# grisetti/g2o_frontend

Hardware: AMD Instinct MI355X
Metric: depth-pair alignments/sec (640x480, 10 GN iters) (higher is better)
Workload: dtype f32; 1 GPU; loop-closure batch: 128 independent 640x480 depth pairs per GPU (u16 mm frames resident in HBM; per pair: convert 2 frames + Aligner::align, 10x1 GN iterations); BASELINE configs[3] shard; mode=pairs, pairs_per_gpu=128, total_pairs=128, rows=480, cols=640, sub_frames=64, sub_pairs=64, streams=4, omega_storage=sym6, step_mode=fused, parallelism=independent pairs sharded over 1 GPU(s), RCCL all-gather of result records only

## Files before the change

### g2o_frontend_amd/csrc/pwn_hip_capi.hip

```cpp
#include <cstdlib>
#include "../../include/pwn_hip.h"
#include "../../include/pwn_hip_testing.h"
#include "pwn_buffers.h"
#include "pwn_kernels.h"
#include "pwn_scene_kernels.h"
#include "pwn_stats.h"

#include <algorithm>
#include <chrono>
#include <condition_variable>
#include <functional>
#include <cstddef>
#include <cstdio>
#include <cstring>
#include <map>
#include <mutex>
#include <string>
#include <thread>
#include <type_traits>
#include <vector>

using namespace pwnhip;

namespace {
// ... 438 lines not shown
  HIPCHK(ctx, ctx->state_host.ensure(B), PWN_HIP_ERR_ALLOCATION);
  HIPCHK(ctx, ctx->counts_host.ensure(B + 1), PWN_HIP_ERR_ALLOCATION);
  HIPCHK(ctx, ctx->match_dev.ensure(B), PWN_HIP_ERR_ALLOCATION);
  HIPCHK(ctx, ctx->match_host.ensure(B), PWN_HIP_ERR_ALLOCATION);
  HIPCHK(ctx, ctx->stats_dev.ensure(B), PWN_HIP_ERR_ALLOCATION);
  HIPCHK(ctx, ctx->stats_host.ensure(B), PWN_HIP_ERR_ALLOCATION);
  ctx->desc_cap = (int)B;
  return PWN_HIP_OK;
}

constexpr int kSinglePassMinFrames = 16;
void launch_stats(const ConvertParams& cp, const FrameDesc* fr, int n, hipStream_t st) {
  const unsigned perFrame = (unsigned)cp.rows * (unsigned)((cp.cols + 255) / 256);
  const unsigned nblk = (n >= 8 ? 8u * (unsigned)((n + 7) / 8) : (unsigned)n) * perFrame;
  hipLaunchKernelGGL(k_stats, dim3(nblk), dim3(256), 0, st, fr, cp, n);
}
int launch_front_end(pwn_hip_ctx* ctx, const ConvertParams& cp, int base, int n, hipStream_t st, bool single_pass, int* fault_out) {
  const FrameDesc* fr = ctx->frames_dev + base;
  if (single_pass) {
    { StageTimer t(ctx, "unproject", st);
      const bool raw = ctx->frames_host[base].raw != nullptr;
      bool aligned = cp.cols % (raw ? 8 : 4) == 0;
      for (int i = 0; i < n && aligned; ++i) {
        const FrameDesc& fd = ctx->frames_host[base + i];
        aligned = ((uintptr_t)(raw ? (const void*)fd.raw : (const void*)fd.depth) & 15u) == 0;
      }
      if (aligned && raw) hipLaunchKernelGGL(k_strip_count<true>, dim3((cp.rows + 3) / 4, n), dim3(256), 0, st, fr, cp);
      else if (aligned) hipLaunchKernelGGL(k_strip_count<false>, dim3((cp.rows + 3) / 4, n), dim3(256), 0, st, fr, cp);
      else hipLaunchKernelGGL(k_strip_count_any, dim3(cp.rows, n), dim3(256), 0, st, fr, cp);
      hipLaunchKernelGGL(k_row_offsets, dim3(n), dim3(1024), 0, st, fr, cp.rows * strips_of(cp.cols)); }
    { StageTimer t(ctx, "integral", st);
      const unsigned epoch = ++ctx->convert_epoch;
      if (epoch == 0) return fail(ctx, PWN_HIP_ERR_LAUNCH, "convert epoch wrapped: recreate the context");
      hipLaunchKernelGGL(k_unproject_integral, dim3(8u * (unsigned)((n + 7) / 8) * (unsigned)strips_of(cp.cols)), dim3(kII_Threads), 0, st, fr, cp, n,
                         epoch, ctx->fault_dev); }
  } else {
    { StageTimer t(ctx, "unproject", st);
      hipLaunchKernelGGL(k_row_count, dim3(cp.rows, n), dim3(256), 0, st, fr, cp);
      hipLaunchKernelGGL(k_row_offsets, dim3(n), dim3(1024), 0, st, fr, cp.rows); }
    { StageTimer t(ctx, "integral_rows", st);
      const unsigned epoch = ++ctx->convert_epoch;
      if (epoch == 0) return fail(ctx, PWN_HIP_ERR_LAUNCH, "convert epoch wrapped: recreate the context");
      hipLaunchKernelGGL(k_unproject_integral_rows, dim3(8u * (unsigned)((bands_of(cp.rows) + 7) / 8) * (unsigned)strips_of(cp.cols), n), dim3(256), 0, st, fr, cp,
                         epoch, ctx->fault_dev); }
    { StageTimer t(ctx, "integral_cols", st);
      hipLaunchKernelGGL(k_integral_cols, dim3((cp.cols + kIC_Block - 1) / kIC_Block, kIntegralChannels, n), dim3(kIC_Block), 0, st, fr, cp.rows, cp.cols,
                         (const int*)ctx->fault_dev, fault_out); }
  }
  return PWN_HIP_OK;
}
int launch_convert(pwn_hip_ctx* ctx, const ConvertParams& cp, int base, int n, hipStream_t st, int* fault_out = nullptr) {
  if (int rc = launch_front_end(ctx, cp, base, n, st, n >= kSinglePassMinFrames, fault_out)) return rc;
  { StageTimer t(ctx, "stats", st);
    launch_stats(cp, ctx->frames_dev + base, n, st); }
  HIPCHK(ctx, hipGetLastError(), PWN_HIP_ERR_LAUNCH);
  return PWN_HIP_OK;
}
void fill_frame(pwn_hip_ctx* ctx, int entry, int slot, const float* depth_dev, const CloudDev& cl) {
  FrameDesc& f = ctx->frames_host[entry];
  f.depth = depth_dev; f.raw = nullptr; f.raw_scale = 0.f;
  f.index = ctx->index_ws + (size_t)slot * ctx->N;
  f.interval = ctx->interval_ws + (size_t)slot * ctx->N;
  f.integral = ctx->integral_ws + (size_t)slot * ctx->N * kIntegralChannels;
  f.rowoff = ctx->rowoff_ws + (size_t)slot * ctx->rowoff_slot;
  f.carry = ctx->carry_ws + (size_t)slot * ctx->carry_slot;
  f.cloud = cl;
  f.count_out = nullptr;
}
int ensure_stats(pwn_hip_ctx* ctx, pwn_hip_cloud* c) {
  if (!c->d.St) HIPCHK(ctx, hipMalloc(&c->d.St, sizeof(float) * 16 * (size_t)c->d.capacity), PWN_HIP_ERR_ALLOCATION);
  return PWN_HIP_OK;
}
int ensure_omega_n(pwn_hip_ctx* ctx, pwn_hip_cloud* c) {
  if (!c->d.OmN) HIPCHK(ctx, hipMalloc((void**)&c->d.OmN, (size_t)c->d.capacity * 9 * sizeof(float)), PWN_HIP_ERR_ALLOCATION);
  return PWN_HIP_OK;
}
void drop_omega_n(pwn_hip_cloud* c) {
  if (c->d.OmN) { (void)hipFree(c->d.OmN); c->d.OmN = nullptr; }
}
int counts_enqueue(pwn_hip_ctx* ctx, int n) {
// ... 52 lines not shown
  for (int i = 0; i < n && aligned; ++i) aligned = ((uintptr_t)ctx->scale_host[base + i].src & 15u) == 0;
  if (aligned) {
    const int dpl = (raw ? 8 : 4) / sc.step;
    const dim3 grid((unsigned)(((size_t)sc.orows * (size_t)((sc.ocols + dpl - 1) / dpl) + 255) / 256), (unsigned)n);
    if (!raw) hipLaunchKernelGGL((k_depth_scale_batch<float, 2>), grid, dim3(256), 0, st, fr, sc.srows, sc.scols, raw_scale, sc.maxCov);
    else if (sc.step == 2) hipLaunchKernelGGL((k_depth_scale_batch<uint16_t, 2>), grid, dim3(256), 0, st, fr, sc.srows, sc.scols, raw_scale, sc.maxCov);
    else hipLaunchKernelGGL((k_depth_scale_batch<uint16_t, 4>), grid, dim3(256), 0, st, fr, sc.srows, sc.scols, raw_scale, sc.maxCov);
  } else {
    const dim3 grid((unsigned)(((size_t)sc.orows * sc.ocols + 255) / 256), (unsigned)n);
    if (raw) hipLaunchKernelGGL(k_depth_scale_batch_any<uint16_t>, grid, dim3(256), 0, st, fr, sc.srows, sc.scols, sc.step, raw_scale, sc.maxCov);
    else hipLaunchKernelGGL(k_depth_scale_batch_any<float>, grid, dim3(256), 0, st, fr, sc.srows, sc.scols, sc.step, raw_scale, sc.maxCov);
  }
  HIPCHK(ctx, hipGetLastError(), PWN_HIP_ERR_LAUNCH);
  return PWN_HIP_OK;
}
struct ConvertJob {
  ConvertParams cp;
  int n = 0, rows = 0, cols = 0;
  size_t N = 0;
  size_t srcN = 0;
  ScaleSpec scale;
  bool raw = false, host_input = false, direct = false;
  float depth_scale = 0.f;
  std::vector<const void*> src;
  std::vector<int> slot;
};
template <typename SRC>
int convert_prepare(pwn_hip_ctx* ctx, const pwn_hip_converter_params* p, const SRC* const* frames, float depth_scale, int n, int rows, int cols,
                    pwn_hip_cloud* const* clouds, int keep_stats, bool want_interval, const std::vector<int>& slot, bool direct, ConvertJob& job,
                    const ScaleSpec& sc = ScaleSpec()) {
  const size_t N = (size_t)rows * cols;
  ctx->last_convert_fault = 0;
  ConvertParams cp = make_convert_params(ctx, p, nullptr, rows, cols, keep_stats);
  cp.lean = want_interval ? 0 : 1;
  if (int rc = ensure_desc(ctx, n)) return rc;
  const bool raw = std::is_same<SRC, uint16_t>::value;
  job.n = n; job.rows = rows; job.cols = cols; job.N = N; job.raw = raw; job.depth_scale = depth_scale; job.slot = slot; job.direct = direct;
  job.scale = sc; job.srcN = sc.step ? (size_t)sc.srows * sc.scols : N;
  job.src.assign(n, nullptr);
  for (int i = 0; i < n; ++i) {
    pwn_hip_cloud* c = clouds[i];
    if (!c || !frames[i]) return fail(ctx, PWN_HIP_ERR_INVALID_ARGUMENT, "null frame or cloud");
    if (i == 0) cp.omSym = c->d.omSym;
    else if (c->d.omSym != cp.omSym) return fail(ctx, PWN_HIP_ERR_INVALID_ARGUMENT, "clouds of one convert batch must share one omega storage (exact9 / sym6)");
    cloud_changes(ctx, c);
    if (keep_stats) { if (int rc = ensure_stats(ctx, c)) return rc; }
    c->has_stats = keep_stats != 0;
    c->n_gauss = 0;
    if (c->d.OmN) { HIPCHK(ctx, hipStreamSynchronize(ctx->stream), PWN_HIP_ERR_LAUNCH); drop_omega_n(c); }
    make_omega_n_classes(p, c->d);
    job.src[i] = frames[i];
    const float* depth_dev = nullptr;
    if (sc.step) depth_dev = ctx->scaled_ws + (size_t)slot[i] * ctx->N;
    else if (!raw) depth_dev = reinterpret_cast<const float*>(frames[i]);
    fill_frame(ctx, i, slot[i], depth_dev, c->d);
    if (c->idximg.cap < N) {
      HIPCHK(ctx, hipStreamSynchronize(ctx->stream), PWN_HIP_ERR_LAUNCH);
      HIPCHK(ctx, c->idximg.ensure(N), PWN_HIP_ERR_ALLOCATION);
    }
    ctx->frames_host[i].index = c->idximg;
    c->idx_valid = cp.hasOffset == 0;
    c->idx_key = index_key(p, rows, cols);
    if (sc.step) {
      ctx->scale_host[i].src = frames[i];
      ctx->scale_host[i].dst = ctx->scaled_ws + (size_t)slot[i] * ctx->N;
    } else if (raw) {
      ctx->frames_host[i].raw = reinterpret_cast<const uint16_t*>(frames[i]);
// ... 68 lines not shown
      }
      HIPCHK(ctx, hipStreamWaitEvent(ctx->copy_stream, ctx->fork_ev, 0), PWN_HIP_ERR_LAUNCH);
    }
    for (int base = 0, k = 0; base < n; base += sub, ++k) {
      const int m = std::min(sub, n - base);
      hipStream_t st = plan.stream(k);
      if (job.host_input) {
        hipStream_t cs = ahead ? ctx->copy_stream : st;
        if (ahead && k >= plan.ns) HIPCHK(ctx, hipStreamWaitEvent(cs, ctx->sync_events[2 * (k - plan.ns) + 1], 0), PWN_HIP_ERR_LAUNCH);
        if (int rc = convert_stage_frames(ctx, job, base, m, cs)) return rc;
        if (ahead) {
          HIPCHK(ctx, hipEventRecord(ctx->sync_events[2 * k], cs), PWN_HIP_ERR_LAUNCH);
          HIPCHK(ctx, hipStreamWaitEvent(st, ctx->sync_events[2 * k], 0), PWN_HIP_ERR_LAUNCH);
        }
      }
      if (int rc = convert_enqueue(ctx, job, base, m, st, direct ? ctx->counts_host + n : nullptr)) return rc;
      if (ahead) HIPCHK(ctx, hipEventRecord(ctx->sync_events[2 * k + 1], st), PWN_HIP_ERR_LAUNCH);
    }
    if (int rc = plan_join(ctx, plan)) return rc;
    return convert_finish(ctx, job, clouds);
  });
}

template <typename SRC>
int debug_front_end_impl(pwn_hip_ctx* ctx, const pwn_hip_converter_params* p, const SRC* const* frames, float depth_scale, int n, int rows, int cols,
                         bool single_pass, int lean, pwn_hip_cloud* const* clouds, float* integral_out, int* index_out, int* interval_out, int* rowoff_out) {
  ctx->stages.clear();
  std::vector<int> slot((size_t)n);
  for (int i = 0; i < n; ++i) slot[i] = i;
  const bool direct = !single_pass && n < kSinglePassMinFrames;
  ConvertJob job;
  if (int rc = convert_prepare<SRC>(ctx, p, frames, depth_scale, n, rows, cols, clouds, 0, lean == 0, slot, direct, job)) return rc;
  if (job.host_input) { if (int rc = convert_stage_frames(ctx, job, 0, n, ctx->stream)) return rc; }
  if (!lean) for (int i = 0; i < n; ++i) {
    HIPCHK(ctx, hipMemsetAsync(clouds[i]->d.Nc, 0, sizeof(float4) * (size_t)clouds[i]->d.capacity, ctx->stream), PWN_HIP_ERR_COPY);
    HIPCHK(ctx, hipMemsetAsync(clouds[i]->d.Om, 0, sizeof(float) * om_floats(clouds[i]->d), ctx->stream), PWN_HIP_ERR_COPY);
  }
  if (int rc = launch_front_end(ctx, job.cp, 0, n, ctx->stream, single_pass, direct ? ctx->counts_host + n : nullptr)) return rc;
  HIPCHK(ctx, hipGetLastError(), PWN_HIP_ERR_LAUNCH);
  const size_t N = job.N, noff = (size_t)rows * (size_t)(single_pass ? strips_of(cols) : 1);
  for (int i = 0; i < n; ++i) {
    const FrameDesc& f = ctx->frames_host[i];
    HIPCHK(ctx, copy_any(integral_out + (size_t)i * N * kIntegralChannels, f.integral, N * kIntegralChannels * sizeof(float), ctx->stream), PWN_HIP_ERR_COPY);
    HIPCHK(ctx, copy_any(index_out + (size_t)i * N, f.index, N * sizeof(int), ctx->stream), PWN_HIP_ERR_COPY);
    HIPCHK(ctx, copy_any(rowoff_out + (size_t)i * noff, f.rowoff, noff * sizeof(int), ctx->stream), PWN_HIP_ERR_COPY);
    if (!lean) HIPCHK(ctx, copy_any(interval_out + (size_t)i * N, f.interval, N * sizeof(int), ctx->stream), PWN_HIP_ERR_COPY);
  }
  if (int rc = convert_finish(ctx, job, clouds)) return rc;
  if (lean) for (int i = 0; i < n; ++i) { clouds[i]->n_host = 0; clouds[i]->idx_valid = false; }
  return PWN_HIP_OK;
}

template <typename SRC>
int depth_scale_batch_impl(pwn_hip_ctx* ctx, const SRC* const* src, float depth_scale, int n, int rows, int cols, int step, float max_depth_cov,
                           float* const* dst, float min_d = 0.f, float max_d = 0.f, int* valid = nullptr) {
  if (!ctx || !src || (!dst && !valid) || n < 0) return fail(ctx, PWN_HIP_ERR_INVALID_ARGUMENT, "null argument");
  ScaleSpec sc;
  if (int rc = make_scale_spec(ctx, rows, cols, step, max_depth_cov, sc)) return rc;
  for (int i = 0; i < n; ++i) if (!src[i] || (dst && !dst[i])) return fail(ctx, PWN_HIP_ERR_INVALID_ARGUMENT, "null frame");
  if (int rc = absorb_copies(ctx)) return rc;
  if (int rc = ensure_scale(ctx, std::min(n, ctx->max_batch))) return rc;
  ctx->stages.clear();
  const bool raw = std::is_same<SRC, uint16_t>::value;
  const size_t sbytes = (size_t)rows * cols * sizeof(SRC), obytes = (size_t)sc.orows * sc.ocols * sizeof(float);
  for (int base = 0; base < n; base += ctx->max_batch) {
    const int m = std::min(ctx->max_batch, n - base);
// ... 834 lines not shown
  HIPCHK(ctx, hipGetLastError(), PWN_HIP_ERR_LAUNCH);
  if (index_image) HIPCHK(ctx, copy_any(index_image, ctx->frames_host[0].index, N * 4, ctx->stream), PWN_HIP_ERR_COPY);
  cloud->has_stats = false;
  pwn_hip_cloud* arr[1] = { cloud };
  return sync_and_counts(ctx, arr, 1);
}
int pwn_hip_project_intervals(pwn_hip_ctx* ctx, const pwn_hip_converter_params* p, const float* depth, int rows, int cols, int* interval_image) {
  if (!ctx || !p || !depth || !interval_image) return fail(ctx, PWN_HIP_ERR_INVALID_ARGUMENT, "null argument");
  if (int rc = check_image(ctx, rows, cols)) return rc;
  const size_t N = (size_t)rows * cols;
  const ConvertParams cp = make_convert_params(ctx, p, nullptr, rows, cols, 0);
  const float* d = nullptr;
  if (int rc = stage_depth(ctx, depth, N, &d)) return rc;
  CloudDev none; std::memset(&none, 0, sizeof(none)); none.count = ctx->scratch_count; none.capacity = 0;
  fill_frame(ctx, 0, 0, d, none);
  HIPCHK(ctx, hipMemcpyAsync(ctx->frames_dev, ctx->frames_host, sizeof(FrameDesc), hipMemcpyHostToDevice, ctx->stream), PWN_HIP_ERR_COPY);
  hipLaunchKernelGGL(k_row_count, dim3(rows, 1), dim3(256), 0, ctx->stream, ctx->frames_dev, cp);
  hipLaunchKernelGGL(k_row_offsets, dim3(1), dim3(1024), 0, ctx->stream, ctx->frames_dev, rows);
  hipLaunchKernelGGL(k_unproject, dim3(rows, 1), dim3(256), 0, ctx->stream, ctx->frames_dev, cp);
  HIPCHK(ctx, hipGetLastError(), PWN_HIP_ERR_LAUNCH);
  HIPCHK(ctx, copy_any(interval_image, ctx->frames_host[0].interval, N * 4, ctx->stream), PWN_HIP_ERR_COPY);
  HIPCHK(ctx, hipStreamSynchronize(ctx->stream), PWN_HIP_ERR_LAUNCH);
  return PWN_HIP_OK;
}
int pwn_hip_integral_image(pwn_hip_ctx* ctx, const int* index_image, const pwn_hip_cloud* cloud, int rows, int cols, float* out) {
  if (!ctx || !index_image || !cloud || !out) return fail(ctx, PWN_HIP_ERR_INVALID_ARGUMENT, "null argument");
  if (int rc = check_image(ctx, rows, cols)) return rc;
  if (int rc = absorb_copies(ctx)) return rc;
  const size_t N = (size_t)rows * cols;
  fill_frame(ctx, 0, 0, nullptr, cloud->d);
  HIPCHK(ctx, copy_any(ctx->frames_host[0].index, index_image, N * 4, ctx->stream), PWN_HIP_ERR_COPY);
  HIPCHK(ctx, hipMemcpyAsync(ctx->frames_dev, ctx->frames_host, sizeof(FrameDesc), hipMemcpyHostToDevice, ctx->stream), PWN_HIP_ERR_COPY);
  hipLaunchKernelGGL(k_integral_rows, dim3((rows + kIR_Rows - 1) / kIR_Rows, 1), dim3(256), 0, ctx->stream, ctx->frames_dev, rows, cols);
  hipLaunchKernelGGL(k_integral_cols, dim3((cols + kIC_Block - 1) / kIC_Block, kIntegralChannels, 1), dim3(kIC_Block), 0, ctx->stream, ctx->frames_dev, rows, cols, (const int*)nullptr, (int*)nullptr);
  HIPCHK(ctx, hipGetLastError(), PWN_HIP_ERR_LAUNCH);
  HIPCHK(ctx, copy_any(out, ctx->frames_host[0].integral, N * kIntegralChannels * 4, ctx->stream), PWN_HIP_ERR_COPY);
  HIPCHK(ctx, hipStreamSynchronize(ctx->stream), PWN_HIP_ERR_LAUNCH);
  return PWN_HIP_OK;
}
int pwn_hip_convert(pwn_hip_ctx* ctx, const pwn_hip_converter_params* p, const float* depth, int rows, int cols, pwn_hip_cloud* cloud,
                    int* index_image, int* interval_image, int keep_stats) {
  const float* frames[1] = { depth };
  pwn_hip_cloud* clouds[1] = { cloud };
  if (int rc = convert_batch_impl<float>(ctx, p, frames, 0.f, 1, rows, cols, clouds, keep_stats, interval_image != nullptr)) return rc;
  const size_t N = (size_t)rows * cols;
  if (index_image) HIPCHK(ctx, hipMemcpy(index_image, ctx->frames_host[0].index, N * 4, hipMemcpyDefault), PWN_HIP_ERR_COPY);
  if (interval_image) HIPCHK(ctx, hipMemcpy(interval_image, ctx->frames_host[0].interval, N * 4, hipMemcpyDefault), PWN_HIP_ERR_COPY);
  return PWN_HIP_OK;
}
int pwn_hip_convert_scaled(pwn_hip_ctx* ctx, const pwn_hip_converter_params* p, const float* depth, int rows, int cols, int step, float max_depth_cov,
                           pwn_hip_cloud* cloud) {
  if (!ctx || !p || !depth || !cloud || step <= 0) return fail(ctx, PWN_HIP_ERR_INVALID_ARGUMENT, "bad argument");
  if (int rc = check_image(ctx, rows, cols)) return rc;
  const int orows = rows / step, ocols = cols / step;
  if (orows <= 0 || ocols <= 0) return fail(ctx, PWN_HIP_ERR_INVALID_ARGUMENT, "scaled image has zero size");
  if (int rc = absorb_copies(ctx)) return rc;
  const size_t n = (size_t)rows * cols, on = (size_t)orows * ocols;
  const float* src = depth;
  if (!is_device_ptr(depth)) { HIPCHK(ctx, hipMemcpyAsync(ctx->depth_ws, depth, n * 4, hipMemcpyHostToDevice, ctx->stream), PWN_HIP_ERR_COPY); src = ctx->depth_ws; }
  float* scaled = ctx->io_ws;
  hipLaunchKernelGGL(k_depth_scale, dim3((unsigned)((on + 255) / 256)), dim3(256), 0, ctx->stream, src, rows, cols, step, max_depth_cov, scaled);
  HIPCHK(ctx, hipGetLastError(), PWN_HIP_ERR_LAUNCH);
  const float* frames[1] = { scaled };
  pwn_hip_cloud* clouds[1] = { cloud };
  return convert_batch_impl<float>(ctx, p, frames, 0.f, 1, orows, ocols, clouds, 0);
}
static void async_convert_loop(AsyncConvert* a, int device) {
// ... 839 lines not shown
```

### g2o_frontend_amd/csrc/pwn_kernels.h

```cpp
#pragma once

#include <hip/hip_runtime.h>
#include <stdint.h>
#include <type_traits>
#include "pwn_math.h"

namespace pwnhip {

constexpr int kMaxIter = 64;
constexpr int kIntegralChannels = 10;
constexpr int kAccN = 37;
constexpr int kPixPerThread = 8;
constexpr int kAlignBlock = 256;
constexpr unsigned long long kZEmpty = ~0ull;
constexpr unsigned kZTag0 = 0xFEu;
constexpr int kZ64IndexBits = 25, kZ64TagShift = 56;
constexpr int kMaxCloudPoints = 1 << kZ64IndexBits;
constexpr int kZIndexBits = 21;
constexpr int kMaxAlignerPoints = 1 << kZIndexBits;
__host__ __device__ __forceinline__ unsigned long long zkey(unsigned tag, float d, int i) {
  return ((unsigned long long)tag << kZ64TagShift) | ((unsigned long long)(__builtin_bit_cast(unsigned, d) & 0x7fffffffu) << kZ64IndexBits) | (unsigned)i;
}
__host__ __device__ __forceinline__ int zkey_index(unsigned long long k, unsigned tag) {
  return ((unsigned)(k >> kZ64TagShift) == tag) ? (int)(k & ((1u << kZ64IndexBits) - 1u)) : -1;
// ... 29 lines not shown
__host__ __device__ __forceinline__ int normal_class(float nx, float ny, float nz, float curvature, float thr) {
  return (nx != 0.f || ny != 0.f || nz != 0.f) ? ((curvature < thr) ? 1 : 2) : 0;
}

struct FrameDesc {
  const float* depth;
  const uint16_t* raw;
  float raw_scale;
  int* index;
  int* interval;
  float* integral;
  int* rowoff;
  unsigned long long* carry;
  CloudDev cloud;
  int* count_out;
};

struct ConvertParams {
  int rows, cols;
  Mat4 iKRt;
  float ivx, ivy;
  float minD, maxD;
  int minRadius, maxRadius, minPoints;
  float statsCurvThr, pointInfoCurvThr, normalInfoCurvThr;
  float pFlat[3], pNonFlat[3];
  int hasOffset;
  Mat4 offset;
  int keepStats;
  int spinLimit;
  int dbgWithhold;
  int omSym;
  int lean;
};

struct PairState {
  Mat4 T;
  Mat4 invTcorr;
  Mat4 invTcorrPrev;
  Mat4 invT;
  Mat4 KRt;
  Mat4 KRtLast;
  Mat4 KRtCur;
  int   it;
  int   pad[3];
  float chi2[kMaxIter];
  int   inliers[kMaxIter];
  int   ncorr[kMaxIter];
  int   ncand[kMaxIter];
};

struct PairDesc {
  CloudDev ref, cur;
  unsigned* zref;
  unsigned* zcur;
  int* curidx;
  const int* refidx0;
  double* partials;
  PairState* state;
  PairState* state_out;
  int* fault;
  unsigned* zdepth;
};

struct AlignParams {
  int rows, cols;
  Mat3 K;
// ... 1 lines not shown
  float minD, maxD;
  float sqDist, normalThr, flatThr, minRatio, maxRatio;
  float maxChi2;
  int robust;
  int settleGuard;
};

__device__ __forceinline__ float wave_sum(float v) {
#pragma unroll
  for (int off = 32; off > 0; off >>= 1) v += __shfl_xor(v, off, 64);
  return v;
}
template <int CTRL, int ROW_MASK> __device__ __forceinline__ float dpp_f32(float v) {
  return __int_as_float(__builtin_amdgcn_update_dpp(0, __float_as_int(v), CTRL, ROW_MASK, 0xF, false));
}
__device__ __forceinline__ float wave_sum_dpp_lane63(float v) {
  v += dpp_f32<0xB1, 0xF>(v);
  v += dpp_f32<0x4E, 0xF>(v);
  v += dpp_f32<0x141, 0xF>(v);
  v += dpp_f32<0x140, 0xF>(v);
  v += dpp_f32<0x142, 0xA>(v);
  v += dpp_f32<0x143, 0xC>(v);
  return v;
}
__device__ __forceinline__ int lane_id() { return threadIdx.x & 63; }
template <typename T> using gptr = T __attribute__((address_space(1)))*;
template <typename T> __device__ __forceinline__ gptr<T> as_global(T* p) { return (gptr<T>)(uintptr_t)p; }
typedef float v4f __attribute__((ext_vector_type(4)));
typedef unsigned v4u __attribute__((ext_vector_type(4)));
__device__ __forceinline__ float4 load4(gptr<const v4f> p) { const v4f v = *p; return make_float4(v.x, v.y, v.z, v.w); }
__device__ __forceinline__ void store4(gptr<v4f> p, const float4 v) { v4f t; t.x = v.x; t.y = v.y; t.z = v.z; t.w = v.w; *p = t; }
typedef float v3f_raw __attribute__((ext_vector_type(3)));
typedef v3f_raw v3f __attribute__((aligned(4)));
__device__ __forceinline__ float4 load_xyz(gptr<const float> p3, unsigned i) { const v3f_raw v = *(gptr<const v3f>)(p3 + 3u * i); return make_float4(v.x, v.y, v.z, 0.f); }
__device__ __forceinline__ float4 load_xyz(const float* p3, int i) { return load_xyz(as_global(p3), (unsigned)i); }
__device__ __forceinline__ void store_xyz(float* p3, int i, float x, float y, float z) { v3f_raw v; v.x = x; v.y = y; v.z = z; *(gptr<v3f>)(as_global(p3) + 3u * (unsigned)i) = v; }
__device__ __forceinline__ void cloud_get(const CloudDev& c, int i, float4& P, float4& Nm) {
  P = load_xyz(c.P3, i);
  const float4 nc = c.Nc[i];
  P.w = nc.w;
  Nm = make_float4(nc.x, nc.y, nc.z, __int_as_float(normal_class(nc.x, nc.y, nc.z, nc.w, c.clsThr)));
}
__device__ __forceinline__ void cloud_put(const CloudDev& c, int i, const float4 P, const float4 Nm) {
  store_xyz(c.P3, i, P.x, P.y, P.z);
  c.Nc[i] = make_float4(Nm.x, Nm.y, Nm.z, P.w);
}
__device__ __forceinline__ float uniform(float v) { return __int_as_float(__builtin_amdgcn_readfirstlane(__float_as_int(v))); }
__device__ __forceinline__ Mat4 uniform_iso(const Mat4& T) {
  Mat4 r;
#pragma unroll
  for (int c = 0; c < 4; ++c) {
    r(0,c) = uniform(T(0,c)); r(1,c) = uniform(T(1,c)); r(2,c) = uniform(T(2,c));
  }
  r(3,0) = 0.f; r(3,1) = 0.f; r(3,2) = 0.f; r(3,3) = 1.f;
  return r;
}

__device__ __forceinline__ Mat4 uniform_iso_global(gptr<const float> m) {
  Mat4 r;
#pragma unroll
  for (int c = 0; c < 4; ++c) {
    r(0,c) = uniform(m[4 * c]); r(1,c) = uniform(m[4 * c + 1]); r(2,c) = uniform(m[4 * c + 2]);
  }
  r(3,0) = 0.f; r(3,1) = 0.f; r(3,2) = 0.f; r(3,3) = 1.f;
  return r;
}
// ... 294 lines not shown
    for (int k = 0; k < kIntegralChannels; ++k) tile[(k * kIR_Rows + lr) * kIR_Stride + lc] = v[k];
  }
  __syncthreads();
  if (tid < kII_Chains) {
    float carry = 0.f;
    if (s > 0) {
      const unsigned long long* src = f.carry + ((size_t)(s - 1) * NB + band) * kII_Chains + tid;
      unsigned long long w = __hip_atomic_load(src, __ATOMIC_RELAXED, __HIP_MEMORY_SCOPE_AGENT);
      int spins = 0;
      while ((unsigned)(w >> 32) != epoch) {
        if (++spins >= cp.spinLimit) { atomicOr(fault, 1); break; }
        __builtin_amdgcn_s_sleep(1);
        w = __hip_atomic_load(src, __ATOMIC_RELAXED, __HIP_MEMORY_SCOPE_AGENT);
      }
      carry = __uint_as_float((unsigned)w);
    }
    const int srow = tid % kIR_Rows, sch = tid / kIR_Rows;
    float* t = &tile[(sch * kIR_Rows + srow) * kIR_Stride];
#pragma unroll 1
    for (int c0 = 0; c0 < kIR_Cols; c0 += 16) {
      float vals[16];
#pragma unroll
      for (int c = 0; c < 16; ++c) vals[c] = t[c0 + c];
#pragma unroll
      for (int c = 0; c < 16; ++c) { carry = vals[c] + carry; vals[c] = carry; }
#pragma unroll
      for (int c = 0; c < 16; ++c) t[c0 + c] = vals[c];
    }
    if (s + 1 < S && (s * NB + band) * kII_Chains + tid != cp.dbgWithhold)
      __hip_atomic_store(f.carry + ((size_t)s * NB + band) * kII_Chains + tid,
                         ((unsigned long long)epoch << 32) | (unsigned long long)__float_as_uint(carry), __ATOMIC_RELAXED, __HIP_MEMORY_SCOPE_AGENT);
  }
  __syncthreads();
#pragma unroll
  for (int j = 0; j < kIR_Rows / 4; ++j) {
    const int lr = wave + 4 * j, lc = lane;
    const int r = r0 + lr, c = x0 + lc;
    if (r < rows && c < cols) {
#pragma unroll
      for (int k = 0; k < kIntegralChannels; ++k)
        f.integral[k * N + (size_t)r * cols + c] = tile[(k * kIR_Rows + lr) * kIR_Stride + lc];
    }
  }
}
constexpr int kSpinLimit = 1 << 20;
__host__ __device__ __forceinline__ int strips_of(int cols) { return (cols + kIR_Cols - 1) / kIR_Cols; }
__host__ __device__ __forceinline__ int bands_of(int rows) { return (rows + kIR_Rows - 1) / kIR_Rows; }

template <bool RAW>
__global__ void __launch_bounds__(256) k_strip_count(const FrameDesc* __restrict__ frames, ConvertParams cp) {
  const FrameDesc& f = frames[blockIdx.y];
  const int wave = threadIdx.x >> 6, lane = lane_id();
  const int r = blockIdx.x * 4 + wave, S = strips_of(cp.cols);
  if (r >= cp.rows) return;
  constexpr int PX = RAW ? 8 : 4;
  constexpr int LPS = kIR_Cols / PX;
  const float scale = f.raw_scale;
  for (int c0 = 0; c0 < cp.cols; c0 += 64 * PX) {
    const int c = c0 + lane * PX;
    int cnt = 0;
    if (c < cp.cols) {
      float d[PX];
      if (RAW) {
        const v4u w = *(gptr<const v4u>)(as_global(f.raw) + ((size_t)r * cp.cols + c));
        const unsigned u[4] = { w.x, w.y, w.z, w.w };
#pragma unroll
// ... 3 lines not shown
        }
      } else {
        const v4f w = *(gptr<const v4f>)(as_global(f.depth) + ((size_t)r * cp.cols + c));
        d[0] = w.x; d[1] = w.y; d[2] = w.z; d[3] = w.w;
      }
#pragma unroll
      for (int k = 0; k < PX; ++k) cnt += depth_in_range(d[k], cp.minD, cp.maxD);
    }
#pragma unroll
    for (int off = 1; off < LPS; off <<= 1) cnt += __shfl_xor(cnt, off, 64);
    const int s = c / kIR_Cols;
    if ((lane & (LPS - 1)) == 0 && c < cp.cols) f.rowoff[r * S + s] = cnt;
  }
}
__global__ void __launch_bounds__(256) k_strip_count_any(const FrameDesc* __restrict__ frames, ConvertParams cp) {
  const FrameDesc& f = frames[blockIdx.y];
  const int r = blockIdx.x, S = strips_of(cp.cols);
  const int wave = threadIdx.x >> 6, lane = lane_id();
  for (int s = wave; s < S; s += 4) {
    const int c = s * kIR_Cols + lane;
    const float d = (c < cp.cols) ? frame_depth(f, (size_t)r * cp.cols + c) : 0.f;
    const bool valid = c < cp.cols && depth_in_range(d, cp.minD, cp.maxD);
    const unsigned long long bal = __ballot(valid);
    if (lane == 0) f.rowoff[r * S + s] = __popcll(bal);
  }
}

__device__ __forceinline__ void lds_barrier() {
  __builtin_amdgcn_fence(__ATOMIC_RELEASE, "workgroup", "local");
  __builtin_amdgcn_s_barrier();
  __builtin_amdgcn_fence(__ATOMIC_ACQUIRE, "workgroup", "local");
}
constexpr int kII_Threads = 320;
__device__ __forceinline__ void unproject_integral_body(const FrameDesc& f, const ConvertParams& cp, const int s, const unsigned epoch, int* __restrict__ fault) {
  const int rows = cp.rows, cols = cp.cols;
  const int S = strips_of(cols), NB = bands_of(rows);
  __shared__ float tile[kIntegralChannels * kIR_Rows * kIR_Stride];
  __shared__ float stage[2][kIR_Rows * kIR_Cols];
  __shared__ int sbase[2][kIR_Rows];
  __shared__ float cin[kII_Chains];
  const int tid = threadIdx.x, lane = tid & 63;
  const int wave = __builtin_amdgcn_readfirstlane(tid >> 6);
  const size_t N = (size_t)rows * cols;
  const int x0 = s * kIR_Cols, c = x0 + lane;
  const bool loader = wave == 4;
  const bool chain = tid < kII_Chains;
  const gptr<const float> gdepth = as_global(f.depth);
  const gptr<const uint16_t> graw = as_global(f.raw);
  const bool is_raw = f.raw != nullptr;
  const float raw_scale = f.raw_scale;
  const gptr<const int> growoff = as_global((const int*)f.rowoff);
  const gptr<int> gindex = as_global(f.index), ginterval = as_global(f.interval);
  const gptr<float> gintegral = as_global(f.integral);
  float* const gP3 = f.cloud.P3;
  const gptr<unsigned long long> gcarry = as_global(f.carry);
  const int capacity = f.cloud.capacity;
  const bool lean = cp.lean != 0;
  float vcarry[3] = { 0.f, 0.f, 0.f };
  bool starved = false;

  unsigned bits[kIR_Rows]; int off = 0;
  auto request_band = [&](int b) {
    const int r0 = b * kIR_Rows;
    if (is_raw) {
#pragma unroll
      for (int i = 0; i < kIR_Rows; ++i) {
        const int r = r0 + i;
        const unsigned pix = (r < rows && c < cols) ? (unsigned)(r * cols + c) : 0u;
        bits[i] = graw[pix];
      }
    } else {
#pragma unroll
      for (int i = 0; i < kIR_Rows; ++i) {
        const int r = r0 + i;
        const unsigned pix = (r < rows && c < cols) ? (unsigned)(r * cols + c) : 0u;
        bits[i] = __float_as_uint(gdepth[pix]);
      }
    }
    const int rr = r0 + (lane & (kIR_Rows - 1));
    off = growoff[(rr < rows ? rr : 0) * S + s];
  };
  auto stage_band = [&](int b) {
    const int r0 = b * kIR_Rows;
#pragma unroll
    for (int i = 0; i < kIR_Rows; ++i) {
      float d;
      if (is_raw) d = raw_to_metres(bits[i], raw_scale);
      else d = __uint_as_float(bits[i]);
      stage[b & 1][i * kIR_Cols + lane] = (r0 + i < rows && c < cols) ? d : 0.f;
    }
    sbase[b & 1][lane & (kIR_Rows - 1)] = off;
// ... 44 lines not shown
            if (idx < capacity) {
              if (!lean) store_xyz(gP3, idx, p.x, p.y, p.z);
              point_channels(v, p.x, p.y, p.z);
            }
            if (!lean) itv = depth_interval(cp.ivx, cp.ivy, dd);
          }
          __builtin_nontemporal_store(idx, gindex + (unsigned)(r * cols + c));
          if (!lean) __builtin_nontemporal_store(itv, ginterval + (unsigned)(r * cols + c));
        }
#pragma unroll
        for (int k = 0; k < kIntegralChannels; ++k) tile[(k * kIR_Rows + lr) * kIR_Stride + lane] = v[k];
      }
    }
    lds_barrier();
    if (chain) {
      float carry = (s > 0) ? cin[tid] : 0.f;
      float* t = &tile[tid * kIR_Stride];
#pragma unroll 1
      for (int c0 = 0; c0 < kIR_Cols; c0 += 16) {
        float vals[16];
#pragma unroll
        for (int cc = 0; cc < 16; ++cc) vals[cc] = t[c0 + cc];
#pragma unroll
        for (int cc = 0; cc < 16; ++cc) { carry = vals[cc] + carry; vals[cc] = carry; }
#pragma unroll
        for (int cc = 0; cc < 16; ++cc) t[c0 + cc] = vals[cc];
      }
      if (s + 1 < S && (s * NB + band) * kII_Chains + tid != cp.dbgWithhold)
        __hip_atomic_store(gcarry + ((size_t)s * NB + band) * kII_Chains + tid,
                           ((unsigned long long)epoch << 32) | (unsigned long long)__float_as_uint(carry),
                           __ATOMIC_RELAXED, __HIP_MEMORY_SCOPE_AGENT);
    }
    lds_barrier();
    if (!loader) {
#pragma unroll
      for (int jj = 0; jj < 3; ++jj) {
        const int q = tid + 256 * jj;
        if (q < kIntegralChannels * kIR_Cols) {
          const int ch = q >> 6;
          float vals[kIR_Rows];
#pragma unroll
          for (int r = 0; r < kIR_Rows; ++r) vals[r] = tile[(ch * kIR_Rows + r) * kIR_Stride + lane];
          float vc = vcarry[jj];
#pragma unroll
          for (int r = 0; r < kIR_Rows; ++r) { vc = vals[r] + vc; vals[r] = vc; }
          vcarry[jj] = vc;
          if (c < cols) {
            const gptr<float> dst = gintegral + ((size_t)ch * N + (size_t)r0 * cols + c);
#pragma unroll
            for (int r = 0; r < kIR_Rows; ++r) if (r0 + r < rows) __builtin_nontemporal_store(vals[r], dst + (unsigned)(r * cols));
          }
        }
      }
    }
    lds_barrier();
  }
}
__global__ void __launch_bounds__(kII_Threads) k_unproject_integral(const FrameDesc* __restrict__ frames, ConvertParams cp, int nframes,
                                                                    unsigned epoch, int* __restrict__ fault) {
  const int S = strips_of(cp.cols);
  const unsigned j = blockIdx.x >> 3;
  const int fi = 8 * (int)(j / (unsigned)S) + (int)(blockIdx.x & 7u), s = (int)(j % (unsigned)S);
  if (fi >= nframes) return;
  unproject_integral_body(frames[fi], cp, s, epoch, fault);
}
constexpr int kIC_Block = 64;
__global__ void __launch_bounds__(kIC_Block) k_integral_cols(const FrameDesc* __restrict__ frames, int rows, int cols, const int* __restrict__ fault,
                                                             int* __restrict__ fault_out) {
  if (fault_out && blockIdx.x == 0 && blockIdx.y == 0 && blockIdx.z == 0 && threadIdx.x == 0) *fault_out = *fault;
  const FrameDesc& f = frames[blockIdx.z];
  const int c = blockIdx.x * kIC_Block + threadIdx.x;
  if (c >= cols) return;
  float* p = f.integral + (size_t)blockIdx.y * rows * cols + c;
  float carry = 0.f;
  int r = 0;
  constexpr int U = 16;
  for (; r + U <= rows; r += U) {
    float v[U];
#pragma unroll
    for (int k = 0; k < U; ++k) v[k] = p[(size_t)(r + k) * cols];
#pragma unroll
    for (int k = 0; k < U; ++k) { carry = v[k] + carry; v[k] = carry; }
#pragma unroll
    for (int k = 0; k < U; ++k) p[(size_t)(r + k) * cols] = v[k];
  }
  for (; r < rows; ++r) { carry = p[(size_t)r * cols] + carry; p[(size_t)r * cols] = carry; }
}

__device__ __forceinline__ int clampi(int v, int lo, int hi) { v = (v < lo) ? lo : v; v = (v > hi) ? hi : v; return v; }
template <typename PTR> __device__ __forceinline__ auto stream_load(PTR p) -> std::remove_cv_t<std::remove_reference_t<decltype(*p)>> {
  return __builtin_nontemporal_load(p);
}
template <typename PTR, typename T> __device__ __forceinline__ void stream_store(PTR p, T v) { __builtin_nontemporal_store(v, p); }
__device__ __forceinline__ v3f_raw stream_load3(gptr<const float> p) { return __builtin_nontemporal_load((gptr<const v3f>)p); }
__device__ __forceinline__ void stream_store3(gptr<float> p, v3f_raw v) { __builtin_nontemporal_store(v, (gptr<v3f>)p); }

__device__ __forceinline__ void stats_pixel(const FrameDesc& f, const ConvertParams& cp, const int r, const int c) {
  const int rows = cp.rows, cols = cp.cols;
  const size_t N = (size_t)rows * cols;
  const gptr<const int> gindex = as_global((const int*)f.index), ginterval = as_global((const int*)f.interval);
  const gptr<const float> gintegral = as_global((const float*)f.integral);
  const gptr<float> gP = as_global(f.cloud.P3), gN = as_global((float*)f.cloud.Nc), gOm = as_global(f.cloud.Om);
  const int cap = f.cloud.capacity;
  const unsigned upix = (unsigned)(r * cols + c);
  const int idx = stream_load(gindex + upix);
  if (idx < 0 || idx >= cap) return;
  int itv;
  float4 P;
  if (cp.lean) {
    float d;
    if (f.raw) d = raw_to_metres(stream_load(as_global(f.raw) + upix), f.raw_scale);
    else d = stream_load(as_global(f.depth) + upix);
    const Vec3 p = unproject_pixel(cp.iKRt, c, r, d);
    P.x = p.x; P.y = p.y; P.z = p.z; P.w = 0.f;
    itv = depth_interval(cp.ivx, cp.ivy, d);
  } else {
    itv = stream_load(ginterval + upix);
    const v3f_raw pv = stream_load3((gptr<const float>)gP + 3u * (unsigned)idx); P.x = pv.x; P.y = pv.y; P.z = pv.z; P.w = 0.f;
  }
  float nx = 0.f, ny = 0.f, nz = 0.f;
  float curvature = 0.f;
  int cls = 0;
  float om[9];
#pragma unroll
  for (int k = 0; k < 9; ++k) om[k] = 0.f;
  float U[9] = { 1.f, 0.f, 0.f, 0.f, 1.f, 0.f, 0.f, 0.f, 1.f };
  float ev[3] = { 0.f, 0.f, 0.f };
  float mean[3] = { 0.f, 0.f, 0.f };
  int npts = 0;
  if (itv >= 0) {
    int rad = itv;
    if (rad < cp.minRadius) rad = cp.minRadius;
    if (rad > cp.maxRadius) rad = cp.maxRadius;
    const int xmin = clampi(c - rad - 1, 0, cols - 1), xmax = clampi(c + rad - 1, 0, cols - 1);
    const int ymin = clampi(r - rad - 1, 0, rows - 1), ymax = clampi(r + rad - 1, 0, rows - 1);
    const unsigned oA = (unsigned)(ymax * cols + xmax), oB = (unsigned)(ymin * cols + xmin);
    const unsigned oC = (unsigned)(ymax * cols + xmin), oD = (unsigned)(ymin * cols + xmax);
    float a[kIntegralChannels];
#pragma unroll
    for (int k = 0; k < kIntegralChannels; ++k) {
      const gptr<const char> pl = (gptr<const char>)(gintegral + (size_t)k * N);
      float v;
      v = *(gptr<const float>)(pl + 4u * oA);
      v = v + *(gptr<const float>)(pl + 4u * oB);
      v = v - *(gptr<const float>)(pl + 4u * oC);
      v = v - *(gptr<const float>)(pl + 4u * oD);
      a[k] = v;
    }
    const int n = (int)a[3];
    if (n >= cp.minPoints) {
      npts = n;
      float d = a[3];
      float c00 = 0, c10 = 0, c20 = 0, c11 = 0, c21 = 0, c22 = 0;
      if (d != 0.f) {
        d = 1.0f / d;
        mean[0] = a[0] * d; mean[1] = a[1] * d; mean[2] = a[2] * d;
        c00 = a[4] * d - mean[0] * mean[0];
        c10 = a[5] * d - mean[1] * mean[0];
        c20 = a[6] * d - mean[2] * mean[0];
        c11 = a[7] * d - mean[1] * mean[1];
        c21 = a[8] * d - mean[2] * mean[1];
        c22 = a[9] * d - mean[2] * mean[2];
      }
      Vec3 v0, v1, v2;
      eig3_direct(c00, c10, c20, c11, c21, c22, ev, v0, v1, v2);
      if (ev[0] < 0.0f) ev[0] = 0.0f;
      U[0] = v0.x; U[1] = v0.y; U[2] = v0.z; U[3] = v1.x; U[4] = v1.y; U[5] = v1.z; U[6] = v2.x; U[7] = v2.y; U[8] = v2.z;
      curvature = (float)((double)ev[0] / ((double)(ev[0] + ev[1] + ev[2]) + 1e-9));
      if (curvature < cp.statsCurvThr) {
        nx = v0.x; ny = v0.y; nz = v0.z;
        const float dp = dot4seq(nx, P.x, ny, P.y, nz, P.z, 0.f, 1.f);
        if (dp > 0) { nx = -nx; ny = -ny; nz = -nz; }
      }
    }
  }
  const float sq = dot4seq(nx, nx, ny, ny, nz, nz, 0.f, 0.f);
  if (sq > 0) {
    float dg[3];
    if (curvature < cp.pointInfoCurvThr) { dg[0] = cp.pFlat[0]; dg[1] = cp.pFlat[1]; dg[2] = cp.pFlat[2]; }
    else { dg[0] = 1.0f / ev[0]; dg[1] = 1.0f / ev[1]; dg[2] = 1.0f / ev[2]; }
#pragma unroll
    for (int i = 0; i < 3; ++i)
#pragma unroll
// ... 855 lines not shown
```

Measured before the change: 12010 alignments/s.

## Interleave integral-image channels into grouped vec4/vec2 planes for vector corner loads

In lean convert mode the ten integral-image channels are now stored as three interleaved groups (4+4+2 floats per pixel) instead of ten separate planes. The integral producers write the grouped layout with vector nontemporal stores, and the stats kernel reads each corner with a single vec4/vec2 load. The second and third groups are fetched only when the point count passes minPoints. This is meant to cut scattered 4-byte gathers in the stats stage and the number of memory transactions, at the cost of a new layout path, strided grouped writes in the rows kernel, and uneven per-wave work in the y-pass where only three waves scan.

```diff
diff --git a/g2o_frontend_amd/csrc/pwn_hip_capi.hip b/g2o_frontend_amd/csrc/pwn_hip_capi.hip
--- a/g2o_frontend_amd/csrc/pwn_hip_capi.hip
+++ b/g2o_frontend_amd/csrc/pwn_hip_capi.hip
@@ -494,8 +494,9 @@
     { StageTimer t(ctx, "integral", st);
       const unsigned epoch = ++ctx->convert_epoch;
       if (epoch == 0) return fail(ctx, PWN_HIP_ERR_LAUNCH, "convert epoch wrapped: recreate the context");
-      hipLaunchKernelGGL(k_unproject_integral, dim3(8u * (unsigned)((n + 7) / 8) * (unsigned)strips_of(cp.cols)), dim3(kII_Threads), 0, st, fr, cp, n,
-                         epoch, ctx->fault_dev); }
+      const dim3 grid(8u * (unsigned)((n + 7) / 8) * (unsigned)strips_of(cp.cols));
+      if (cp.lean == kLeanGrouped) hipLaunchKernelGGL(k_unproject_integral_grouped, grid, dim3(kII_Threads), 0, st, fr, cp, n, epoch, ctx->fault_dev);
+      else hipLaunchKernelGGL(k_unproject_integral, grid, dim3(kII_Threads), 0, st, fr, cp, n, epoch, ctx->fault_dev); }
   } else {
     { StageTimer t(ctx, "unproject", st);
       hipLaunchKernelGGL(k_row_count, dim3(cp.rows, n), dim3(256), 0, st, fr, cp);
@@ -506,8 +507,10 @@
       hipLaunchKernelGGL(k_unproject_integral_rows, dim3(8u * (unsigned)((bands_of(cp.rows) + 7) / 8) * (unsigned)strips_of(cp.cols), n), dim3(256), 0, st, fr, cp,
                          epoch, ctx->fault_dev); }
     { StageTimer t(ctx, "integral_cols", st);
-      hipLaunchKernelGGL(k_integral_cols, dim3((cp.cols + kIC_Block - 1) / kIC_Block, kIntegralChannels, n), dim3(kIC_Block), 0, st, fr, cp.rows, cp.cols,
-                         (const int*)ctx->fault_dev, fault_out); }
+      const bool grouped = cp.lean == kLeanGrouped;
+      const dim3 grid = grouped ? dim3((ig_width(0) * cp.cols + kIC_Block - 1) / kIC_Block, kIG_Groups, n)
+                                   : dim3((cp.cols + kIC_Block - 1) / kIC_Block, kIntegralChannels, n);
+      hipLaunchKernelGGL(k_integral_cols, grid, dim3(kIC_Block), 0, st, fr, cp.rows, cp.cols, (const int*)ctx->fault_dev, fault_out, grouped ? 1 : 0); }
   }
   return PWN_HIP_OK;
 }
@@ -626,7 +629,7 @@
   const size_t N = (size_t)rows * cols;
   ctx->last_convert_fault = 0;
   ConvertParams cp = make_convert_params(ctx, p, nullptr, rows, cols, keep_stats);
-  cp.lean = want_interval ? 0 : 1;
+  cp.lean = want_interval ? 0 : kLeanGrouped;
   if (int rc = ensure_desc(ctx, n)) return rc;
   const bool raw = std::is_same<SRC, uint16_t>::value;
   job.n = n; job.rows = rows; job.cols = cols; job.N = N; job.raw = raw; job.depth_scale = depth_scale; job.slot = slot; job.direct = direct;
@@ -761,6 +764,7 @@
   ConvertJob job;
   if (int rc = convert_prepare<SRC>(ctx, p, frames, depth_scale, n, rows, cols, clouds, 0, lean == 0, slot, direct, job)) return rc;
   if (job.host_input) { if (int rc = convert_stage_frames(ctx, job, 0, n, ctx->stream)) return rc; }
+  if (lean) job.cp.lean = 1;
   if (!lean) for (int i = 0; i < n; ++i) {
     HIPCHK(ctx, hipMemsetAsync(clouds[i]->d.Nc, 0, sizeof(float4) * (size_t)clouds[i]->d.capacity, ctx->stream), PWN_HIP_ERR_COPY);
     HIPCHK(ctx, hipMemsetAsync(clouds[i]->d.Om, 0, sizeof(float) * om_floats(clouds[i]->d), ctx->stream), PWN_HIP_ERR_COPY);
@@ -1661,7 +1665,7 @@
   HIPCHK(ctx, copy_any(ctx->frames_host[0].index, index_image, N * 4, ctx->stream), PWN_HIP_ERR_COPY);
   HIPCHK(ctx, hipMemcpyAsync(ctx->frames_dev, ctx->frames_host, sizeof(FrameDesc), hipMemcpyHostToDevice, ctx->stream), PWN_HIP_ERR_COPY);
   hipLaunchKernelGGL(k_integral_rows, dim3((rows + kIR_Rows - 1) / kIR_Rows, 1), dim3(256), 0, ctx->stream, ctx->frames_dev, rows, cols);
-  hipLaunchKernelGGL(k_integral_cols, dim3((cols + kIC_Block - 1) / kIC_Block, kIntegralChannels, 1), dim3(kIC_Block), 0, ctx->stream, ctx->frames_dev, rows, cols, (const int*)nullptr, (int*)nullptr);
+  hipLaunchKernelGGL(k_integral_cols, dim3((cols + kIC_Block - 1) / kIC_Block, kIntegralChannels, 1), dim3(kIC_Block), 0, ctx->stream, ctx->frames_dev, rows, cols, (const int*)nullptr, (int*)nullptr, 0);
   HIPCHK(ctx, hipGetLastError(), PWN_HIP_ERR_LAUNCH);
   HIPCHK(ctx, copy_any(out, ctx->frames_host[0].integral, N * kIntegralChannels * 4, ctx->stream), PWN_HIP_ERR_COPY);
   HIPCHK(ctx, hipStreamSynchronize(ctx->stream), PWN_HIP_ERR_LAUNCH);
diff --git a/g2o_frontend_amd/csrc/pwn_kernels.h b/g2o_frontend_amd/csrc/pwn_kernels.h
--- a/g2o_frontend_amd/csrc/pwn_kernels.h
+++ b/g2o_frontend_amd/csrc/pwn_kernels.h
@@ -85,6 +85,10 @@
   int omSym;
   int lean;
 };
+constexpr int kLeanGrouped = 2;
+constexpr int kIG_Groups = 3;
+__host__ __device__ constexpr int ig_width(int g) { return g < 2 ? 4 : 2; }
+__host__ __device__ __forceinline__ size_t ig_at(size_t N, int g, size_t pix) { return (size_t)4 * (size_t)g * N + pix * (size_t)ig_width(g); }
 
 struct PairState {
   Mat4 T;
@@ -152,6 +156,8 @@
 __device__ __forceinline__ void store4(gptr<v4f> p, const float4 v) { v4f t; t.x = v.x; t.y = v.y; t.z = v.z; t.w = v.w; *p = t; }
 typedef float v3f_raw __attribute__((ext_vector_type(3)));
 typedef v3f_raw v3f __attribute__((aligned(4)));
+typedef v4f ig4 __attribute__((aligned(8)));
+typedef float ig2 __attribute__((ext_vector_type(2)));
 __device__ __forceinline__ float4 load_xyz(gptr<const float> p3, unsigned i) { const v3f_raw v = *(gptr<const v3f>)(p3 + 3u * i); return make_float4(v.x, v.y, v.z, 0.f); }
 __device__ __forceinline__ float4 load_xyz(const float* p3, int i) { return load_xyz(as_global(p3), (unsigned)i); }
 __device__ __forceinline__ void store_xyz(float* p3, int i, float x, float y, float z) { v3f_raw v; v.x = x; v.y = y; v.z = z; *(gptr<v3f>)(as_global(p3) + 3u * (unsigned)i) = v; }
@@ -512,6 +518,18 @@
                          ((unsigned long long)epoch << 32) | (unsigned long long)__float_as_uint(carry), __ATOMIC_RELAXED, __HIP_MEMORY_SCOPE_AGENT);
   }
   __syncthreads();
+  if (cp.lean == kLeanGrouped) {
+    for (int g = 0; g < kIG_Groups; ++g) {
+      const int w = ig_width(g), rowlen = kIR_Cols * w;
+      for (int j = tid; j < kIR_Rows * rowlen; j += 256) {
+        const int lr = j / rowlen, e = j % rowlen;
+        const int lc = e / w, k = e % w;
+        const int r = r0 + lr, c = x0 + lc;
+        if (r < rows && c < cols) f.integral[ig_at(N, g, (size_t)r * cols + c) + k] = tile[((4 * g + k) * kIR_Rows + lr) * kIR_Stride + lc];
+      }
+    }
+    return;
+  }
 #pragma unroll
   for (int j = 0; j < kIR_Rows / 4; ++j) {
     const int lr = wave + 4 * j, lc = lane;
@@ -581,6 +599,33 @@
   __builtin_amdgcn_fence(__ATOMIC_ACQUIRE, "workgroup", "local");
 }
 constexpr int kII_Threads = 320;
+constexpr int kIG_RowBatch = 4;
+static_assert(kIR_Rows % kIG_RowBatch == 0, "row batch");
+template <int W>
+__device__ __forceinline__ void ypass_group(const float* tile, const int ch0, const int lane, float (&vc)[4], const bool incol, const gptr<float> dst,
+                                            const unsigned rowFloats, const int r0, const int rows) {
+#pragma unroll
+  for (int rb = 0; rb < kIR_Rows; rb += kIG_RowBatch) {
+    float vals[kIG_RowBatch][W];
+#pragma unroll
+    for (int r = 0; r < kIG_RowBatch; ++r)
+#pragma unroll
+      for (int k = 0; k < W; ++k) vals[r][k] = tile[((ch0 + k) * kIR_Rows + rb + r) * kIR_Stride + lane];
+#pragma unroll
+    for (int r = 0; r < kIG_RowBatch; ++r)
+#pragma unroll
+      for (int k = 0; k < W; ++k) { vc[k] = vals[r][k] + vc[k]; vals[r][k] = vc[k]; }
+    if (incol) {
+#pragma unroll
+      for (int r = 0; r < kIG_RowBatch; ++r) if (r0 + rb + r < rows) {
+        const gptr<float> q = dst + (unsigned)(rb + r) * rowFloats;
+        if (W == 4) { v4f v; v.x = vals[r][0]; v.y = vals[r][1]; v.z = vals[r][2]; v.w = vals[r][3]; __builtin_nontemporal_store(v, (gptr<ig4>)q); }
+        else { ig2 v; v.x = vals[r][0]; v.y = vals[r][W - 1]; __builtin_nontemporal_store(v, (gptr<ig2>)q); }
+      }
+    }
+  }
+}
+template <bool GROUPED>
 __device__ __forceinline__ void unproject_integral_body(const FrameDesc& f, const ConvertParams& cp, const int s, const unsigned epoch, int* __restrict__ fault) {
   const int rows = cp.rows, cols = cp.cols;
   const int S = strips_of(cols), NB = bands_of(rows);
@@ -604,8 +649,8 @@
   float* const gP3 = f.cloud.P3;
   const gptr<unsigned long long> gcarry = as_global(f.carry);
   const int capacity = f.cloud.capacity;
-  const bool lean = cp.lean != 0;
-  float vcarry[3] = { 0.f, 0.f, 0.f };
+  const bool lean = GROUPED || cp.lean != 0;
+  float vcarry[GROUPED ? 4 : 3] = {};
   bool starved = false;
 
   unsigned bits[kIR_Rows]; int off = 0;
@@ -716,7 +761,13 @@
                            __ATOMIC_RELAXED, __HIP_MEMORY_SCOPE_AGENT);
     }
     lds_barrier();
-    if (!loader) {
+    if constexpr (GROUPED) {
+      if (wave < kIG_Groups) {
+        const gptr<float> dst = gintegral + ig_at(N, wave, (size_t)r0 * cols + c);
+        if (wave < 2) ypass_group<4>(tile, 4 * wave, lane, vcarry, c < cols, dst, 4u * (unsigned)cols, r0, rows);
+        else ypass_group<2>(tile, 8, lane, vcarry, c < cols, dst, 2u * (unsigned)cols, r0, rows);
+      }
+    } else if (!loader) {
 #pragma unroll
       for (int jj = 0; jj < 3; ++jj) {
         const int q = tid + 256 * jj;
@@ -746,16 +797,26 @@
   const unsigned j = blockIdx.x >> 3;
   const int fi = 8 * (int)(j / (unsigned)S) + (int)(blockIdx.x & 7u), s = (int)(j % (unsigned)S);
   if (fi >= nframes) return;
-  unproject_integral_body(frames[fi], cp, s, epoch, fault);
+  unproject_integral_body<false>(frames[fi], cp, s, epoch, fault);
+}
+__global__ void __launch_bounds__(kII_Threads) k_unproject_integral_grouped(const FrameDesc* __restrict__ frames, ConvertParams cp, int nframes,
+                                                                            unsigned epoch, int* __restrict__ fault) {
+  const int S = strips_of(cp.cols);
+  const unsigned j = blockIdx.x >> 3;
+  const int fi = 8 * (int)(j / (unsigned)S) + (int)(blockIdx.x & 7u), s = (int)(j % (unsigned)S);
+  if (fi >= nframes) return;
+  unproject_integral_body<true>(frames[fi], cp, s, epoch, fault);
 }
 constexpr int kIC_Block = 64;
-__global__ void __launch_bounds__(kIC_Block) k_integral_cols(const FrameDesc* __restrict__ frames, int rows, int cols, const int* __restrict__ fault,
-                                                             int* __restrict__ fault_out) {
+__global__ void __launch_bounds__(kIC_Block) k_integral_cols(const FrameDesc* __restrict__ frames, int rows, int cols_, const int* __restrict__ fault,
+                                                             int* __restrict__ fault_out, int grouped) {
   if (fault_out && blockIdx.x == 0 && blockIdx.y == 0 && blockIdx.z == 0 && threadIdx.x == 0) *fault_out = *fault;
   const FrameDesc& f = frames[blockIdx.z];
+  const size_t N = (size_t)rows * cols_;
+  const int cols = grouped ? ig_width((int)blockIdx.y) * cols_ : cols_;
   const int c = blockIdx.x * kIC_Block + threadIdx.x;
   if (c >= cols) return;
-  float* p = f.integral + (size_t)blockIdx.y * rows * cols + c;
+  float* p = f.integral + (grouped ? ig_at(N, (int)blockIdx.y, 0) : (size_t)blockIdx.y * N) + c;
   float carry = 0.f;
   int r = 0;
   constexpr int U = 16;
@@ -821,18 +882,35 @@
     const unsigned oA = (unsigned)(ymax * cols + xmax), oB = (unsigned)(ymin * cols + xmin);
     const unsigned oC = (unsigned)(ymax * cols + xmin), oD = (unsigned)(ymin * cols + xmax);
     float a[kIntegralChannels];
-#pragma unroll
-    for (int k = 0; k < kIntegralChannels; ++k) {
-      const gptr<const char> pl = (gptr<const char>)(gintegral + (size_t)k * N);
-      float v;
-      v = *(gptr<const float>)(pl + 4u * oA);
-      v = v + *(gptr<const float>)(pl + 4u * oB);
-      v = v - *(gptr<const float>)(pl + 4u * oC);
-      v = v - *(gptr<const float>)(pl + 4u * oD);
-      a[k] = v;
+    const gptr<const char> g0 = (gptr<const char>)gintegral, g1 = (gptr<const char>)(gintegral + ig_at(N, 1, 0)), g2 = (gptr<const char>)(gintegral + ig_at(N, 2, 0));
+    if (cp.lean == kLeanGrouped) {
+      const v4f A = *(gptr<const ig4>)(g0 + 16u * oA), B = *(gptr<const ig4>)(g0 + 16u * oB);
+      const v4f C = *(gptr<const ig4>)(g0 + 16u * oC), D = *(gptr<const ig4>)(g0 + 16u * oD);
+      a[0] = ((A.x + B.x) - C.x) - D.x; a[1] = ((A.y + B.y) - C.y) - D.y; a[2] = ((A.z + B.z) - C.z) - D.z; a[3] = ((A.w + B.w) - C.w) - D.w;
+#pragma unroll
+      for (int k = 4; k < kIntegralChannels; ++k) a[k] = 0.f;
+    } else {
+#pragma unroll
+      for (int k = 0; k < kIntegralChannels; ++k) {
+        const gptr<const char> pl = (gptr<const char>)(gintegral + (size_t)k * N);
+        float v;
+        v = *(gptr<const float>)(pl + 4u * oA);
+        v = v + *(gptr<const float>)(pl + 4u * oB);
+        v = v - *(gptr<const float>)(pl + 4u * oC);
+        v = v - *(gptr<const float>)(pl + 4u * oD);
+        a[k] = v;
+      }
     }
     const int n = (int)a[3];
     if (n >= cp.minPoints) {
+      if (cp.lean == kLeanGrouped) {
+        const v4f A = *(gptr<const ig4>)(g1 + 16u * oA), B = *(gptr<const ig4>)(g1 + 16u * oB);
+        const v4f C = *(gptr<const ig4>)(g1 + 16u * oC), D = *(gptr<const ig4>)(g1 + 16u * oD);
+        const ig2 E = *(gptr<const ig2>)(g2 + 8u * oA), F = *(gptr<const ig2>)(g2 + 8u * oB);
+        const ig2 G = *(gptr<const ig2>)(g2 + 8u * oC), H = *(gptr<const ig2>)(g2 + 8u * oD);
+        a[4] = ((A.x + B.x) - C.x) - D.x; a[5] = ((A.y + B.y) - C.y) - D.y; a[6] = ((A.z + B.z) - C.z) - D.z; a[7] = ((A.w + B.w) - C.w) - D.w;
+        a[8] = ((E.x + F.x) - G.x) - H.x; a[9] = ((E.y + F.y) - G.y) - H.y;
+      }
       npts = n;
       float d = a[3];
       float c00 = 0, c10 = 0, c20 = 0, c11 = 0, c21 = 0, c22 = 0;
```

Result: faster. 12250 alignments/s, median of 6 (+2.0%).
